# alibasaran/die-e

Measured on AMD Instinct MI355X. Metric: self-play games/sec, higher is better.
Workload: dtype bf16

## Files before the change

### die-e_amd/csrc/mcts_kernels.hip

```cpp
#include <hip/hip_runtime.h>
#include <stdint.h>

#include <algorithm>
#include <type_traits>

#include "bg_device.h"
#include "nn_device.h"
#include "launch.h"
#include "mcts_device.h"
#include "search_types.h"
#include "wave_ops.h"

namespace diee {

__device__ __forceinline__ void backprop(const Tree& T, size_t base, uint32_t idx, float v) {
    while (idx != kNone) {
        T.visits[base + idx] += 1.0f;
        T.value[base + idx] += v;
        idx = T.parent[base + idx];
    }
}

__device__ __forceinline__ void backprop_path(const Tree& T, size_t base, uint32_t my_node, int lane, uint32_t len, float v) {
    if ((uint32_t)lane < len) {
// ... 877 lines not shown
            __syncthreads();
        }
        const uint32_t share = ncand < want ? ncand : want, dem = hit ? 0u : 1u;
        mine_rows = dem + share;
        uint32_t start = 0;
        if (lane == 0 && mine_rows) start = atomicAdd(&L.n_rows[A.q], mine_rows);
        start = (uint32_t)__builtin_amdgcn_readfirstlane((int)start);
        if ((uint32_t)lane < mine_rows && start + (uint32_t)lane < L.rows) {
            const uint32_t node = (dem && lane == 0) ? leaf : D.cand[(uint32_t)lane - dem];
            const uint32_t r = A.q * L.rows + start + (uint32_t)lane;
            store_state(&L.rows_state[r], (dem && lane == 0) ? lst : load_state(&T.state[base + node]));
            L.rows_node[r] = (slot << 24) | node;
        }
        uint32_t extra = 0;
        if (second_round) {
            uint32_t unused_;
            const bool met = tail_meet(L.bar2 + A.q, n, true, lane, S.overflow, unused_);
            const uint32_t more = redistribute ? ncand - share : 0u;
            extra = met ? nchild + more : 0u;
            uint32_t start2 = 0;
            if (lane == 0 && extra) {
                start2 = atomicAdd(&L.n_rows[A.q], extra);
                const uint32_t fit = start2 >= L.rows ? 0u : extra < L.rows - start2 ? extra : L.rows - start2;
                if (fit < extra) atomicSub(&L.n_rows[A.q], extra - fit);
            }
            start2 = (uint32_t)__builtin_amdgcn_readfirstlane((int)start2);
            extra = start2 >= L.rows ? 0u : extra < L.rows - start2 ? extra : L.rows - start2;
            for (uint32_t j = (uint32_t)lane; j < extra; j += 64) {
                const uint32_t r = A.q * L.rows + start2 + j;
                if (j < nchild) {
                    BgState cs = lst;
                    int d0, d1;
                    draw_dice(seed, gid, rnd, it + 1u, j, d0, d1);
                    bg_apply_dev(cs, D.ws.play[j], d0, d1);
                    store_state(&L.rows_state[r], cs);
                    L.rows_node[r] = (slot << 24) | (used + j);
                } else {
                    const uint32_t node = D.cand[share + (j - nchild)];
                    store_state(&L.rows_state[r], load_state(&T.state[base + node]));
                    L.rows_node[r] = (slot << 24) | node;
                }
            }
        }
        cn[SC_NN_ROWS] += mine_rows + extra;
        if (lane == 0 && share + extra) atomicAdd(&L.state[3], share + extra);
    }
    if (lane == 0) store_counters(S, slot, cn);
    TL_STAMP(3);
    if (slot == 0 && lane == 0 && !done) L.n_dem[A.q] = misses;
    if (slot == 0 && lane == 0) {
        const uint32_t was = atomicMax(&L.state[1], done ? 1u : 0u);
        const uint32_t now = was > (done ? 1u : 0u) ? was : (done ? 1u : 0u);
        L.state[0] = it;
        if (!done) L.state[2] += 1u;
        L.host[0] = it; L.host[1] = now; L.host[2] = A.q;
        __threadfence_system();
    }
}

constexpr int kFreeSpinFew = 48, kFreeFewGames = 64;
constexpr uint32_t kFreeRowBits = 12;
struct FreeArgs { Free F; uint32_t q; };
#ifdef DIEE_TAIL_STAMPS
__device__ unsigned long long g_free_stamps[16];
#define FR_STAMP(i) do { const unsigned long long tn_ = __builtin_readcyclecounter(); if (threadIdx.x == 0) atomicAdd(&g_free_stamps[i], tn_ - fr_prev_); fr_prev_ = __builtin_readcyclecounter(); } while (0)
#define FR_COUNT(i, k) do { if (threadIdx.x == 0) atomicAdd(&g_free_stamps[i], (unsigned long long)(k)); } while (0)
extern "C" int diee_dev_free_stamps(unsigned long long* out, int reset) {
    if (out && hipMemcpyFromSymbol(out, HIP_SYMBOL(g_free_stamps), sizeof(unsigned long long) * 16) != hipSuccess) return 1;
    if (reset) { unsigned long long z[16] = {0}; if (hipMemcpyToSymbol(HIP_SYMBOL(g_free_stamps), z, sizeof(z)) != hipSuccess) return 1; }
    return 0;
}
#else
#define FR_STAMP(i) do {} while (0)
#define FR_COUNT(i, k) do {} while (0)
#endif
constexpr uint32_t kFreeLdsNodeBytes = 32;
__host__ __device__ __forceinline__ constexpr uint32_t free_hdr(uint32_t meta, uint32_t first_child) {
    return (meta & 0xE0000000u) | (((meta >> 16) & 0x1ffu) << 20) | (first_child & 0xFFFFFu);
}
__host__ __device__ __forceinline__ constexpr uint32_t hdr_nch(uint32_t h) { return (h >> 20) & 0x1ffu; }
__host__ __device__ __forceinline__ constexpr uint32_t hdr_fc(uint32_t h) { return h & 0xFFFFFu; }
__host__ __device__ constexpr size_t free_lds_bytes(uint32_t ln) {
    return (size_t)ln * kFreeLdsNodeBytes + sizeof(WaveScratch) + sizeof(float) * kMaxPlays + sizeof(uint16_t) * kMaxPlays + sizeof(uint32_t) * 64u;
}
struct TreeF {
    const Tree& T; size_t base; uint32_t ln;
    float *lvis, *lval, *lpri; uint32_t* lhdr;
    __device__ __forceinline__ float vis(uint32_t i) const { return i < ln ? lvis[i] : T.visits[base + i]; }
    __device__ __forceinline__ float val(uint32_t i) const { return i < ln ? lval[i] : T.value[base + i]; }
    __device__ __forceinline__ float pri(uint32_t i) const { return i < ln ? lpri[i] : T.prior[base + i]; }
    __device__ __forceinline__ uint32_t hdr(uint32_t i) const { return i < ln ? lhdr[i] : free_hdr(T.meta[base + i], T.first_child[base + i]); }
    __device__ __forceinline__ void add(uint32_t i, float v) const {
        const float nv = vis(i) + 1.0f, nw = val(i) + v;
        if (i < ln) { lvis[i] = nv; lval[i] = nw; }
        T.visits[base + i] = nv; T.value[base + i] = nw;
    }
    __device__ __forceinline__ void set_header(uint32_t i, uint32_t m, uint32_t f) const {
        if (i < ln) lhdr[i] = free_hdr(m, f);
        T.meta[base + i] = m; T.first_child[base + i] = f;
    }
};
__device__ __forceinline__ uint32_t free_load(const uint32_t* p) { return __hip_atomic_load(p, __ATOMIC_RELAXED, __HIP_MEMORY_SCOPE_AGENT); }

__global__ __launch_bounds__(64) void k_free(Tree T, Slots S, Segs G, uint32_t n, SearchParams P, float c, FreeArgs A) {
    extern __shared__ __attribute__((aligned(16))) char free_smem[];
    const uint32_t slot = blockIdx.x;
    if (slot >= n) return;
    const Free& F = A.F;
    const int lane = threadIdx.x;
    if (F.state[0] != 0u) return;
    uint32_t it = F.prog[slot];
    if (it >= F.iterations) { if (lane == 0) F.wish_n[slot] = it << 8; return; }
    const uint32_t active0 = A.q == 0 ? n : F.state[4];
    const uint32_t active = active0 ? active0 : 1u;
    const bool few = active * 8u <= n || active <= 8u;
    const uint32_t iter_cap = few ? 64u * F.iter_cap : F.iter_cap;
#ifdef DIEE_TAIL_STAMPS
    unsigned long long fr_prev_ = __builtin_readcyclecounter();
    const unsigned long long fr_t0_ = fr_prev_;
#endif
    FR_COUNT(8, 1);
    const uint32_t ln = F.lds_nodes;
    float* lvis = (float*)free_smem; float* lval = lvis + ln; float* lpri = lval + ln;
    float* vvis = lpri + ln; float* vval = vvis + ln;
    float* lcval = vval + ln;
    uint32_t* lhdr = (uint32_t*)(lcval + ln); uint32_t* lcrow = lhdr + ln;
    WaveScratch& ws = *reinterpret_cast<WaveScratch*>(lcrow + ln);
    float* raw = reinterpret_cast<float*>(&ws + 1);
    uint16_t* code = reinterpret_cast<uint16_t*>(raw + kMaxPlays);
    uint32_t* cand = reinterpret_cast<uint32_t*>(code + kMaxPlays);
    float* lgs = (float*)&ws.keyA[0];
    const size_t base = (size_t)slot * T.node_cap;
    uint32_t* crow_g = F.crow + base;
    float* cval_g = F.cval + base;
    const TreeF X{T, base, ln, lvis, lval, lpri, lhdr};
    const bool quirks = P.quirks != 0;
    const uint32_t seg = G.n == 1 ? 0u : S.seg[slot];
    const uint32_t seg_first = G.first_slot[seg], seg_end = G.end_slot[seg];
    const unsigned long long seed = G.seed[seg];
    const uint32_t gid = S.game_id[slot], rnd = S.round[slot];
    const float rv0 = S.root_value0[seg];
    unsigned long long evals = S.counters[(size_t)seg * CNT_COUNT + CNT_NN_EVALS];
    uint32_t used = T.used[slot];
    bool lterm = S.leaf_term[slot] != 0;
    uint32_t leaf = S.leaf[slot], sel = S.sel[slot], leaf_meta = S.leaf_meta[slot];
    float sel_value = S.sel_value[slot];
    uint32_t plen = S.path_len[slot];
    uint32_t pnode = S.path[(size_t)slot * kPathCap + lane];
    uint32_t cn[SC_COUNT];
    load_counters(S, slot, cn);
    const BgState rs = load_state(&T.state[base]);
    const int root_player = st_player(rs);
    uint32_t fsel = 0;
    if (A.q == 0) { if (lane == 0) F.first_sel[slot] = sel == kNone ? kNone : 0u; }
    if (quirks && slot == seg_first) {
        uint32_t m = 0;
        for (uint32_t g = seg_first + (uint32_t)lane; g < seg_end; g += 64) {
            const uint32_t f = A.q == 0 ? (S.sel[g] == kNone ? kNone : 0u) : F.first_sel[g];
            m = f == kNone ? 0x7fffffffu : (f > m ? f : m);
            if (f == kNone) break;
        }
        fsel = (uint32_t)wave_allmax_i32((int)m);
    }
    const uint32_t nl = used < ln ? used : ln;
    for (uint32_t i0 = 0; i0 < nl; i0 += 256) {
        float a[4], b[4], p[4], cv4[4]; uint32_t m[4], f[4], r[4];
#pragma unroll
        for (int u = 0; u < 4; ++u) {
            const uint32_t i = i0 + 64u * u + (uint32_t)lane;
            const size_t gi = base + (i < nl ? i : 0u);
            a[u] = T.visits[gi]; b[u] = T.value[gi]; p[u] = T.prior[gi]; m[u] = T.meta[gi]; f[u] = T.first_child[gi]; r[u] = crow_g[i < nl ? i : 0u]; cv4[u] = cval_g[i < nl ? i : 0u];
        }
#pragma unroll
        for (int u = 0; u < 4; ++u) {
            const uint32_t i = i0 + 64u * u + (uint32_t)lane;
            if (i < nl) { lvis[i] = a[u]; lval[i] = b[u]; lpri[i] = p[u]; lhdr[i] = free_hdr(m[u], f[u]); lcrow[i] = r[u]; lcval[i] = cv4[u]; }
        }
    }
    __syncthreads();
    if (A.q > 0) {
        const uint32_t pq = A.q - 1, off = F.grant_off[slot], cnt = F.grant_cnt[slot];
        const size_t rb = (size_t)(pq % F.ring) * F.rows;
        for (uint32_t r = lane; r < cnt; r += 64) {
            const uint32_t row = off + r;
            const uint32_t node = F.rows_idx[rb + row] - (uint32_t)base;
            const float* h = F.hv + (rb + row) * 72;
            float dot = 0.0f;
            for (int i = 0; i < 72; ++i) dot += h[i] * S.wv[i];
            const float cv = tanhf(dot + S.wv[72]);
            const uint32_t id = ((pq << kFreeRowBits) | row) + 1u;
            cval_g[node] = cv; crow_g[node] = id;
            if (node < ln) { lcrow[node] = id; lcval[node] = cv; }
        }
        cn[SC_NN_ROWS] += cnt;
        __syncthreads();
    }
    auto at_hand = [&](uint32_t cr) { return cr != 0u && ((cr - 1u) >> kFreeRowBits) + F.ring >= A.q; };
    auto crow_of = [&](uint32_t i) { return i < ln ? lcrow[i] : crow_g[i]; };
    auto batch_progress = [&]() {
        int m = 0x7fffffff;
        for (uint32_t g = seg_first + (uint32_t)lane; g < seg_end; g += 64) { const int v = (int)free_load(&F.prog[g]); m = v < m ? v : m; }
        return (uint32_t)(-wave_allmax_i32(-m));
    };
    BgState lst = load_state(&S.eval_states[slot]);
    FR_STAMP(0);
    bool have = false, stalled = false;
    uint32_t minprog = 0;
    auto net_row = [&](uint32_t cr_) {
        NetRowLoaded p;
        const size_t ring = (size_t)(((cr_ - 1u) >> kFreeRowBits) % F.ring) * F.rows + ((cr_ - 1u) & ((1u << kFreeRowBits) - 1u));
        p.vh = value_head_load(F.hv + ring * 72, S.wv, lane);
        softmax_load(F.logits + ring * 1352, lane, p.lg);
        return p;
    };
    uint32_t cr = lterm ? 0u : crow_of(leaf);
    NetRowLoaded pre;
    if (!lterm && at_hand(cr)) pre = net_row(cr);
    uint32_t ran = 0;
    for (;; ++ran) {
        have = lterm || at_hand(cr);
        if (!have) break;
        if (ran >= iter_cap) { stalled = true; break; }
        uint32_t* iflag = S.iter_flags + 2 * ((size_t)seg * G.iter_cap + it);
        const bool need_cnt = quirks && slot == seg_first && it < fsel;
        const bool need_any = lterm && (quirks || slot == seg_first);
        uint2 ifl = make_uint2(1u, 0u);
        if (need_any || need_cnt) {
            bool fin = false;
            const int spins = n <= (uint32_t)kFreeFewGames ? kFreeSpinFew : 1;
            for (int spin = 0; spin < spins; ++spin) {
                if (!need_cnt && (iflag[0] != 0u || free_load(&iflag[0]) != 0u)) { ifl.x = 1u; fin = true; break; }
                if (minprog < it) minprog = batch_progress();
                if (minprog >= it) {
                    ifl.x = free_load(&iflag[0]); ifl.y = free_load(&iflag[1]);
                    fin = true;
                    break;
                }
                __builtin_amdgcn_s_sleep(8);
            }
            if (!fin) { stalled = true; break; }
        }
        FR_STAMP(1);
        const bool active = ifl.x != 0u;
        float v = 0.0f;
        bool do_expand = !lterm, do_backprop = true;
        if (active) {
            if (slot == seg_first) evals += (unsigned long long)(seg_end - seg_first);
            if (lterm) {
                do_expand = false; do_backprop = false;
                if (quirks && sel != kNone) {
                    if (plen) { if ((uint32_t)lane < plen) X.add(pnode, sel_value); }
                    else if (lane == 0) { for (uint32_t i = sel; i != kNone; i = T.parent[base + i]) X.add(i, sel_value); }
                }
            } else {
                v = value_head_eval(pre.vh, lane);
                sel_value = v;
            }
            const uint32_t m0 = lterm ? 0u : leaf_meta;
            if (do_expand && !(m0 & kDrained)) {
                int k = bg_legal_plays_wave(lst, &ws, lane, S.overflow);
                if (k > kMaxPlays) { if (lane == 0) atomicOr(S.overflow, 1u); k = 0; }
                const int r0 = st_roll(lst, 0), r1 = st_roll(lst, 1);
                float smM, smInv;
                softmax_reduce(pre.lg, lane, smM, smInv);
#pragma unroll
                for (int q = 0; q < 22; ++q) lgs[lane + 64 * q] = pre.lg[q];
                __syncthreads();
                for (int j = lane; j < k; j += 64) {
                    const uint32_t cd = bg_encode_dev(r0, r1, ws.play[j]);
                    raw[j] = softmax_prob(lgs[cd], smM, smInv); code[j] = (uint16_t)cd;
                }
                __syncthreads();
                float pr[4];
#pragma unroll
                for (int r = 0; r < 4; ++r) pr[r] = lane + 64 * r < k ? raw[lane + 64 * r] : 0.0f;
                float sum = 0.0f;
#pragma unroll
                for (int r = 0; r < 4; ++r) {
                    const int kr = k - 64 * r < 64 ? k - 64 * r : 64;
                    for (int j = 0; j < kr; ++j) sum += __builtin_bit_cast(float, __builtin_amdgcn_readlane(__builtin_bit_cast(int, pr[r]), j));
                }
                const uint32_t first = used;
                if (first + (uint32_t)k > T.node_cap) {
                    if (lane == 0) atomicOr(S.overflow, 2u);
                } else {
                    const uint32_t e = it + 1u;
                    for (int j = lane; j < k; j += 64) {
                        const uint32_t cl = first + (uint32_t)j;
                        const size_t ci = base + cl;
                        BgState cs = lst;
                        int d0, d1;
                        draw_dice(seed, gid, rnd, e, (uint32_t)j, d0, d1);
                        bg_apply_dev(cs, ws.play[j], d0, d1);
                        store_state(&T.state[ci], cs);
                        const float prj = raw[j] / sum;
                        const uint32_t cm = (uint32_t)code[j] | meta_terminal_bits(cs);
                        T.visits[ci] = 0.0f; T.value[ci] = 0.0f; T.prior[ci] = prj;
                        T.parent[ci] = leaf; T.first_child[ci] = 0; T.meta[ci] = cm;
                        crow_g[cl] = 0u;
                        if (cl < ln) { lvis[cl] = 0.0f; lval[cl] = 0.0f; lpri[cl] = prj; lhdr[cl] = free_hdr(cm, 0u); lcrow[cl] = 0; }
                    }
                    const uint32_t nmeta = kDrained | ((uint32_t)k << 16) | (m0 & kMetaKeep);
                    if (lane == 0) X.set_header(leaf, nmeta, first);
                    used = first + (uint32_t)k;
                    cn[SC_EXPANSIONS] += 1; cn[SC_CHILDREN] += (uint32_t)k;
                    if ((uint32_t)k > cn[SC_MAX_CHILDREN]) cn[SC_MAX_CHILDREN] = (uint32_t)k;
                }
                __syncthreads();
            }
            if (do_backprop) {
                if (plen) { if ((uint32_t)lane < plen) X.add(pnode, v); }
                else if (lane == 0) { for (uint32_t i = leaf; i != kNone; i = T.parent[base + i]) X.add(i, v); }
            }
            if (quirks && slot == seg_first && ifl.y != 0u && lane == 0) {
                float rvis = X.vis(0), rval = X.val(0);
                for (uint32_t i = 0; i < ifl.y; ++i) { rvis += 1.0f; rval += rv0; }
                if (ln > 0) { lvis[0] = rvis; lval[0] = rval; }
                T.visits[base] = rvis; T.value[base] = rval;
            }
            __syncthreads();
        }
        FR_STAMP(2);
        uint32_t published = 0;
        if (it + 1 < F.iterations) {
            uint32_t* nflag = S.iter_flags + 2 * ((size_t)seg * G.iter_cap + it + 1);
            uint32_t node = 0, depth = 0, mine = lane == 0 ? 0u : kNone;
            uint32_t mt = X.hdr(0), fcn = hdr_fc(mt);
            float nvis = X.vis(0);
            for (;;) {
                const uint32_t k = hdr_nch(mt);
                if (k == 0) break;
                const float sq = sqrtf(nvis);
                Best b{0.0f, -1};
                int lastnan = -1;
                for (uint32_t j = lane; j < k; j += 64) {
                    const uint32_t ci = fcn + j;
                    const float vis = X.vis(ci), val = X.val(ci), pr = X.pri(ci);
                    const float q = vis == 0.0f ? 0.0f : val / vis;
                    const float t = sq / (vis + 1.0f);
                    const float u = c * t;
                    const float w = u * pr;
                    const float sc_ = q + w;
                    if (sc_ != sc_) lastnan = (int)j;
                    else if (b.j < 0 || !(b.s > sc_)) { b.s = sc_; b.j = (int)j; }
                }
                lastnan = wave_allmax_i32(lastnan);
                if (lastnan >= 0) {
                    b.s = 0.0f; b.j = -1;
                    for (uint32_t j = lane; j < k; j += 64) {
                        if ((int)j <= lastnan) continue;
                        const uint32_t ci = fcn + j;
                        const float vis = X.vis(ci), val = X.val(ci), pr = X.pri(ci);
                        const float q = vis == 0.0f ? 0.0f : val / vis;
                        const float t = sq / (vis + 1.0f);
                        const float u = c * t;
                        const float w = u * pr;
                        const float sc_ = q + w;
                        if (b.j < 0 || !(b.s > sc_)) { b.s = sc_; b.j = (int)j; }
                    }
                }
                b = wave_best(b);
                const int chosen = b.j >= 0 ? b.j : lastnan;
                node = fcn + (uint32_t)chosen;
                ++depth;
                if ((uint32_t)lane == depth) mine = node;
                mt = X.hdr(node); fcn = hdr_fc(mt); nvis = X.vis(node);
            }
            const uint32_t npl = depth < S.path_cap ? depth + 1u : 0u;
            cn[SC_SELECTIONS] += 1; cn[SC_DEPTH_SUM] += depth;
            if (mt & kMetaTerminal) {
                const float tv = ((mt & kMetaWinnerPlus) ? 1 : -1) == root_player ? 1.0f : -1.0f;
                if (npl) { if ((uint32_t)lane < npl) X.add(mine, tv); }
                else if (lane == 0) { for (uint32_t i = node; i != kNone; i = T.parent[base + i]) X.add(i, tv); }
                cn[SC_TERMINAL] += 1;
                lterm = true;
                if (lane == 0 && quirks && sel == kNone) published = atomicAdd(&nflag[1], 1u);
            } else {
                lterm = false; leaf = node; plen = npl; pnode = mine;
                leaf_meta = T.meta[base + node];
                if (lane == 0) {
                    if (nflag[0] == 0u) published = atomicOr(&nflag[0], 1u);
                    if (sel == kNone) F.first_sel[slot] = it + 1u;
                }
                sel = node;
                lst = load_state(&T.state[base + node]);
            }
            cr = lterm ? 0u : crow_of(leaf);
            if (!lterm && at_hand(cr)) pre = net_row(cr);
        }
        ++it;
        __syncthreads();
        if (lane == 0) {
            asm volatile("" :: "v"(published) : "memory");
            atomicExch(&F.prog[slot], it);
        }
        FR_STAMP(3); FR_COUNT(9, 1);
        if (it >= F.iterations) break;
    }
    if (lane == 0) {
        S.leaf_term[slot] = lterm ? 1 : 0; S.leaf[slot] = leaf; S.sel[slot] = sel; S.leaf_meta[slot] = leaf_meta;
        S.sel_value[slot] = sel_value; S.path_len[slot] = (uint8_t)plen;
        T.used[slot] = used;
        if (slot == seg_first) S.counters[(size_t)seg * CNT_COUNT + CNT_NN_EVALS] = evals;
        store_state(&S.eval_states[slot], lst);
    }
    if ((uint32_t)lane < plen) S.path[(size_t)slot * kPathCap + lane] = pnode;
    const bool done = it >= F.iterations;
    uint32_t nw = 0;
    const bool dem = !done && !stalled && !have;
    if (!done) {
        uint32_t* wl = F.wish + (size_t)slot * kFreeWish;
        if (dem) { if (lane == 0) wl[0] = leaf; nw = 1; }
        uint32_t want0 = F.cand_max < kFreeWish - 1u ? F.cand_max : kFreeWish - 1u;
        uint32_t steps_max = F.rollout_steps;
        if (few && want0) {
            const uint32_t room = (F.rows > active ? F.rows - active : 0u) / active;
            want0 = room + 1u < kFreeWish - 1u ? (room + 1u > want0 ? room + 1u : want0) : kFreeWish - 1u;
            steps_max = 2u * F.rollout_steps + 8u;
        }
        const uint32_t want = few ? want0 : (want0 > ran / 2u + 1u ? want0 - ran / 2u : (want0 ? 1u : 0u));
        uint32_t ncand = 0;
        if (want > 0 && steps_max > 0) {
            const uint32_t nu = used < ln ? used : ln;
            for (uint32_t i = lane; i < nu; i += 64) { vvis[i] = lvis[i]; vval[i] = lval[i]; }
            __syncthreads();
            const uint32_t demanded = dem ? leaf : kNone;
            uint32_t fruitless = 0;
            for (uint32_t step = 0; step < steps_max && ncand < want && fruitless < 8; ++step) {
                uint32_t node = 0, depth = 0, mine = lane == 0 ? 0u : kNone, mt = 0;
                for (;;) {
                    mt = X.hdr(node);
                    const uint32_t k = hdr_nch(mt);
                    if (k == 0) break;
                    const uint32_t fcn = hdr_fc(mt);
                    const float sq = __builtin_amdgcn_sqrtf(node < nu ? vvis[node] : T.visits[base + node]);
                    Best b{0.0f, -1};
                    for (uint32_t j = lane; j < k; j += 64) {
                        const uint32_t ci = fcn + j;
                        const float vis = ci < nu ? vvis[ci] : T.visits[base + ci], val = ci < nu ? vval[ci] : T.value[base + ci];
                        const float q = vis == 0.0f ? 0.0f : val * __builtin_amdgcn_rcpf(vis);
                        const float sc_ = q + (c * (sq * __builtin_amdgcn_rcpf(vis + 1.0f))) * X.pri(ci);
                        if (sc_ == sc_ && (b.j < 0 || !(b.s > sc_))) { b.s = sc_; b.j = (int)j; }
                    }
                    b = wave_best(b);
                    node = fcn + (uint32_t)(b.j >= 0 ? b.j : (int)k - 1);
                    ++depth;
                    if ((uint32_t)lane == depth) mine = node;
                    if (depth >= 63) break;
                }
                const uint32_t cr = crow_of(node);
                float x = 0.0f;
                bool fresh = false;
                if (mt & kMetaTerminal) x = ((mt & kMetaWinnerPlus) ? 1 : -1) == root_player ? 1.0f : -1.0f;
                else if (at_hand(cr)) x = node < ln ? lcval[node] : cval_g[node];
                else if (!(mt & kDrained) && node != demanded) fresh = __ballot((uint32_t)lane < ncand && cand[lane] == node) == 0ull;
                if (fresh) { if (lane == 0) { cand[ncand] = node; wl[nw + ncand] = node; } ++ncand; fruitless = 0; } else ++fruitless;
                if ((uint32_t)lane <= depth && mine < nu) { vvis[mine] += 1.0f; vval[mine] += x; }
                __syncthreads();
                FR_COUNT(11, 1);
            }
        }
        nw += ncand;
    }
    if (lane == 0) {
        F.wish_n[slot] = nw | (it << 8) | (dem ? 0x80000000u : 0u);
        store_counters(S, slot, cn);
    }
    FR_STAMP(4);
#ifdef DIEE_TAIL_STAMPS
    if (threadIdx.x == 0) atomicMax(&g_free_stamps[10], __builtin_readcyclecounter() - fr_t0_);
#endif
}

__global__ __launch_bounds__(1024) void k_free_pack(Free F, uint32_t n, uint32_t node_cap, uint32_t q, const BgState* __restrict__ arena) {
    const uint32_t kBoost = F.lag_boost < kFreeBoostMax ? F.lag_boost : kFreeBoostMax, kLagStep = F.lag_step ? F.lag_step : 1u;
    __shared__ uint32_t hist[kFreeWish + kFreeBoostMax + 2];
    __shared__ uint32_t wsum[16];
    __shared__ uint32_t s_full, s_rem, s_dem, s_undone, s_maxprog;
    const int tid = threadIdx.x, lane = tid & 63, wave = tid >> 6;
    if (F.state[0] != 0u) return;
    if (tid < (int)(kFreeWish + kFreeBoostMax + 2)) hist[tid] = 0;
    if (tid == 0) { s_dem = 0; s_undone = 0; s_maxprog = 0; }
    __syncthreads();
    const uint32_t rot = (q * 131u) % n;
    const uint32_t g = (uint32_t)tid < n ? ((uint32_t)tid + rot) % n : 0u;
    const uint32_t w = (uint32_t)tid < n ? F.wish_n[g] : ((F.iterations) << 8);
    const uint32_t cnt = (w & 0xffu) < kFreeWish ? (w & 0xffu) : kFreeWish, dem = (w >> 31) < cnt ? (w >> 31) : cnt, spec = cnt - dem, prog = (w >> 8) & 0x7fffffu;
    const bool undone = prog < F.iterations;
    if ((uint32_t)tid < n && undone) { atomicMax(&s_maxprog, prog); atomicAdd(&s_undone, 1u); if (dem) atomicAdd(&s_dem, 1u); }
    __syncthreads();
    const uint32_t lag = undone ? s_maxprog - prog : 0u;
    const uint32_t shift = kBoost - (lag / kLagStep < kBoost ? lag / kLagStep : kBoost);
    if ((uint32_t)tid < n) for (uint32_t r = 1; r <= spec; ++r) atomicAdd(&hist[r + shift], 1u);
    __syncthreads();
    if (tid == 0) {
        const uint32_t room = F.rows > s_dem ? F.rows - s_dem : 0u;
        uint32_t full = 0, used_rows = 0;
        for (uint32_t k = 1; k <= kFreeWish + kBoost; ++k) {
            if (used_rows + hist[k] > room) break;
            used_rows += hist[k]; full = k;
        }
        s_full = full; s_rem = room - used_rows;
    }
    __syncthreads();
    const uint32_t full = s_full, rem = s_rem;
    const uint32_t whole = full > shift ? (full - shift < spec ? full - shift : spec) : 0u;
    const int more = ((uint32_t)tid < n && spec > whole && whole + 1u + shift == full + 1u) ? 1 : 0;
    int inc = wave_inclusive_scan_i32(more);
    if (lane == 63) wsum[wave] = (uint32_t)inc;
    __syncthreads();
    uint32_t before = 0;
    for (int v = 0; v < wave; ++v) before += wsum[v];
    const uint32_t my_rank = before + (uint32_t)(inc - more);
    __syncthreads();
    const uint32_t grant = (uint32_t)tid < n ? dem + whole + ((more && my_rank < rem) ? 1u : 0u) : 0u;
    inc = wave_inclusive_scan_i32((int)grant);
    if (lane == 63) wsum[wave] = (uint32_t)inc;
    __syncthreads();
    before = 0;
    uint32_t total = 0;
    for (int v = 0; v < 16; ++v) { if (v < wave) before += wsum[v]; total += wsum[v]; }
    const uint32_t off = before + (uint32_t)inc - grant;
    if ((uint32_t)tid < n) {
        const uint32_t fit = off >= F.rows ? 0u : (grant < F.rows - off ? grant : F.rows - off);
        F.grant_off[g] = off; F.grant_cnt[g] = fit;
        uint32_t* out = F.rows_idx + (size_t)(q % F.ring) * F.rows + off;
        const uint32_t* wl = F.wish + (size_t)g * kFreeWish;
        for (uint32_t j = 0; j < fit; ++j) out[j] = g * node_cap + wl[j];
        if (F.rows_state) {
            BgState* so = F.rows_state + (size_t)(q % F.ring) * F.rows + off;
            for (uint32_t j = 0; j < fit; ++j) store_state(&so[j], load_state(&arena[(size_t)g * node_cap + wl[j]]));
        }
    }
    if (tid == 0) {
        if (total > F.rows) total = F.rows;
        F.n_rows[q] = total; F.n_dem[q] = s_dem < total ? s_dem : total;
        const uint32_t all_done = s_undone ? 0u : 1u;
        F.state[0] = all_done; F.state[4] = s_undone;
        if (total) { F.state[1] += 1u; F.state[2] += total - s_dem; }
        F.host[0] = all_done; F.host[1] = q;
        __threadfence_system();
    }
}

__global__ __launch_bounds__(256) void k_reduce_counters(Slots S, Segs G, unsigned long long* step_log, uint32_t step) {
    __shared__ unsigned long long part[SC_COUNT][4];
    const uint32_t seg = blockIdx.x;
    const uint32_t s0 = G.first_slot[seg], s1 = G.end_slot[seg];
    if (s1 <= s0) return;
    const int tid = threadIdx.x, lane = tid & 63, wave = tid >> 6;
    unsigned long long acc[SC_COUNT];
#pragma unroll
    for (int c = 0; c < SC_COUNT; ++c) acc[c] = 0;
    for (uint32_t s = s0 + tid; s < s1; s += 256)
#pragma unroll
        for (int c = 0; c < SC_COUNT; ++c) {
            const unsigned long long v = S.slot_cnt[s * SC_COUNT + c];
            if (c == SC_MAX_CHILDREN) acc[c] = v > acc[c] ? v : acc[c]; else acc[c] += v;
        }
#pragma unroll
    for (int c = 0; c < SC_COUNT; ++c) {
#pragma unroll
        for (int d = 32; d >= 1; d >>= 1) {
            const unsigned long long o = __shfl_xor(acc[c], d);
            if (c == SC_MAX_CHILDREN) acc[c] = o > acc[c] ? o : acc[c]; else acc[c] += o;
        }
        if (lane == 0) part[c][wave] = acc[c];
    }
    __syncthreads();
    if (tid == 0) {
        const int map[SC_COUNT] = {CNT_SELECTIONS, CNT_DEPTH_SUM, CNT_TERMINAL, CNT_EXPANSIONS, CNT_CHILDREN, CNT_MAX_CHILDREN, CNT_ILLEGAL, CNT_NN_ROWS};
        unsigned long long* cnt = S.counters + (size_t)seg * CNT_COUNT;
        for (int c = 0; c < SC_COUNT; ++c) {
            unsigned long long t = 0;
            for (int w = 0; w < 4; ++w) t = c == SC_MAX_CHILDREN ? (part[c][w] > t ? part[c][w] : t) : t + part[c][w];
            if (c == SC_MAX_CHILDREN) { if (t > cnt[map[c]]) cnt[map[c]] = t; }
            else cnt[map[c]] += t;
            if (step_log && c == SC_EXPANSIONS) atomicAdd(&step_log[2 * (size_t)step], t);
            if (step_log && c == SC_NN_ROWS) atomicAdd(&step_log[2 * (size_t)step + 1], t);
        }
    }
}

__global__ __launch_bounds__(1024) void k_row_map(const uint8_t* __restrict__ skip, uint32_t n, uint32_t* __restrict__ row_slot,
                                                  uint32_t* __restrict__ slot_row, uint32_t* __restrict__ n_rows,
                                                  uint32_t* __restrict__ rows_log, uint32_t log_idx) {
    __shared__ uint32_t wsum[16];
    __shared__ uint32_t carry;
    const int tid = threadIdx.x, lane = tid & 63, wave = tid >> 6;
    if (tid == 0) carry = 0;
    __syncthreads();
    for (uint32_t c0 = 0; c0 < n; c0 += 1024) {
        const uint32_t i = c0 + tid;
        const bool keep = i < n && skip[i] == 0;
        const unsigned long long bal = __ballot(keep);
        if (lane == 0) wsum[wave] = (uint32_t)__popcll(bal);
        __syncthreads();
        uint32_t off = carry;
        for (int w = 0; w < wave; ++w) off += wsum[w];
        const uint32_t pos = off + (uint32_t)__popcll(bal & ((1ull << lane) - 1ull));
        if (keep) { row_slot[pos] = i; slot_row[i] = pos; }
        __syncthreads();
        if (tid == 0) { uint32_t t = 0; for (int w = 0; w < 16; ++w) t += wsum[w]; carry += t; }
        __syncthreads();
    }
    if (tid == 0) { *n_rows = carry; if (rows_log) rows_log[log_idx] = carry; }
}

__global__ __launch_bounds__(64) void k_root_probs(Tree T, uint32_t n, float* __restrict__ probs,
                                                   uint32_t* __restrict__ nch, float* __restrict__ root_visits) {
    __shared__ float sum_s;
    const uint32_t slot = blockIdx.x;
    if (slot >= n) return;
    const int lane = threadIdx.x;
    const size_t base = (size_t)slot * T.node_cap;
    const uint32_t k = meta_nch(T.meta[base]), fc = T.first_child[base];
    float* row = probs + (size_t)slot * 1352;
    const float fill = k == 0 ? __uint_as_float(0x7fc00000u) : 0.0f;
    for (int a = lane; a < 1352; a += 64) row[a] = fill;
    if (lane == 0) {
        float s = 0.0f;
        for (uint32_t j = 0; j < k; ++j) s += T.visits[base + fc + j];
        sum_s = s;
        nch[slot] = k;
// ... 118 lines not shown
        Gm.rounds[g] = round + 1;
        atomicAdd(&cnt[CNT_PLIES], 1ull);
        const int w = bg_winner_dev(s);
        if (w != 0) {
            if (!(flushed && !P.quirks)) { Gm.ev_b_count[g] = nf + 1; Gm.ev_b_step[g] = step; }
            Gm.winner[g] = (int8_t)w;
            removed = true;
        }
        if (removed) { Gm.alive[g] = 0; atomicAdd(&cnt[CNT_GAMES], 1ull); }
    }
}

__global__ __launch_bounds__(1024) void k_compact_live(Games Gm, uint32_t n_live, uint32_t n_segs, uint32_t* n_live_out) {
    __shared__ uint32_t wsum[16];
    __shared__ uint32_t carry;
    __shared__ uint32_t per_seg[kMaxSegments];
    const int tid = threadIdx.x, lane = tid & 63, wave = tid >> 6;
    if (tid == 0) carry = 0;
    if (tid < (int)kMaxSegments) per_seg[tid] = 0;
    __syncthreads();
    for (uint32_t c0 = 0; c0 < n_live; c0 += 1024) {
        const uint32_t i = c0 + tid;
        uint32_t g = 0;
        bool keep = false;
        if (i < n_live) { g = Gm.live[i]; keep = Gm.alive[g] != 0; }
        if (keep) atomicAdd(&per_seg[Gm.seg[g]], 1u);
        const unsigned long long bal = __ballot(keep);
        if (lane == 0) wsum[wave] = (uint32_t)__popcll(bal);
        __syncthreads();
        uint32_t off = carry;
        for (int w = 0; w < wave; ++w) off += wsum[w];
        const uint32_t pos = off + (uint32_t)__popcll(bal & ((1ull << lane) - 1ull));
        __syncthreads();
        if (keep) Gm.live[pos] = g;
        __syncthreads();
        if (tid == 0) { uint32_t t = 0; for (int w = 0; w < 16; ++w) t += wsum[w]; carry += t; }
        __syncthreads();
    }
    if (tid == 0) n_live_out[0] = carry;
    if (tid < (int)n_segs) n_live_out[1 + tid] = per_seg[tid];
}

__global__ __launch_bounds__(1024) void k_deliver_scan(Games Gm, Segs G, uint32_t n_live, uint32_t step, DeliverEvent* __restrict__ ev,
                                                       uint32_t* __restrict__ summary) {
    __shared__ uint32_t wrow[16], wev[16];
    __shared__ uint32_t carry_rows, carry_ev;
    __shared__ uint32_t seg_base[kMaxSegments], seg_rows[kMaxSegments], seg_ev0[kMaxSegments], seg_nev[kMaxSegments];
    const int tid = threadIdx.x, lane = tid & 63, wave = tid >> 6;
    if (tid == 0) { carry_rows = 0; carry_ev = 0; }
    if (tid < (int)kMaxSegments) { seg_base[tid] = 0; seg_rows[tid] = 0; seg_ev0[tid] = kNone; seg_nev[tid] = 0; }
    __syncthreads();
    for (uint32_t c0 = 0; c0 < n_live; c0 += 1024) {
        const uint32_t i = c0 + tid;
        uint32_t g = 0, seg = 0, ca = 0, cb = 0;
        if (i < n_live) {
            g = Gm.live[i]; seg = Gm.seg[g];
            const uint32_t a = Gm.ev_a_count[g], b = Gm.ev_b_count[g];
            if (a != kNone && Gm.ev_a_step[g] == step) ca = a;
            if (b != kNone && Gm.ev_b_step[g] == step) cb = b;
        }
        const uint32_t nr = ca + cb, ne = (ca ? 1u : 0u) + (cb ? 1u : 0u);
        uint32_t pr = nr, pe = ne;
#pragma unroll
        for (int d = 1; d < 64; d <<= 1) {
            const uint32_t xr = __shfl_up(pr, d, 64), xe = __shfl_up(pe, d, 64);
            if (lane >= d) { pr += xr; pe += xe; }
        }
        if (lane == 63) { wrow[wave] = pr; wev[wave] = pe; }
        __syncthreads();
        uint32_t off_r = carry_rows, off_e = carry_ev;
        for (int w = 0; w < wave; ++w) { off_r += wrow[w]; off_e += wev[w]; }
        const uint32_t row0 = off_r + pr - nr;
        uint32_t e = off_e + pe - ne;
        if (i < n_live && i == G.first_slot[seg]) seg_base[seg] = row0;
        if (ca) { ev[e] = DeliverEvent{g, ca, row0, seg}; ++e; }
        if (cb) ev[e] = DeliverEvent{g, 0x80000000u | cb, row0 + ca, seg};
        __syncthreads();
        if (tid == 0) { uint32_t tr = 0, te = 0; for (int w = 0; w < 16; ++w) { tr += wrow[w]; te += wev[w]; } carry_rows += tr; carry_ev += te; }
        __syncthreads();
    }
    const uint32_t n_ev = carry_ev;
    for (uint32_t e = tid; e < n_ev; e += 1024) {
        DeliverEvent d = ev[e];
        d.row0 -= seg_base[d.seg];
        ev[e] = d;
        atomicAdd(&seg_rows[d.seg], d.kind_count & 0x7FFFFFFFu);
        atomicMin(&seg_ev0[d.seg], e);
        atomicAdd(&seg_nev[d.seg], 1u);
    }
    __syncthreads();
    if (tid < (int)G.n) {
        summary[DeliverSummary::rows(G.n, tid)] = seg_rows[tid];
        summary[DeliverSummary::ev0(G.n, tid)] = seg_nev[tid] ? seg_ev0[tid] : 0u;
        summary[DeliverSummary::nev(G.n, tid)] = seg_nev[tid];
    }
}

__global__ __launch_bounds__(256) void k_deliver_copy(Games Gm, Segs G, const DeliverEvent* __restrict__ ev, uint32_t n_ev, uint32_t r0,
                                                      uint32_t r1, DeliverOut out) {
    for (uint32_t r = r0 + blockIdx.x; r < r1; r += gridDim.x) {
        uint32_t lo = 0, hi = n_ev;
        while (hi - lo > 1) { const uint32_t mid = (lo + hi) >> 1; if (ev[mid].row0 <= r) lo = mid; else hi = mid; }
        const DeliverEvent d = ev[lo];
        const uint32_t fr = r - d.row0;
        const size_t s = (size_t)d.g * Gm.frag_cap + fr, o = (size_t)(r - r0);
        for (int a = threadIdx.x; a < 1352 / 4; a += 256)
            reinterpret_cast<float4*>(out.ps + o * 1352)[a] = reinterpret_cast<const float4*>(Gm.frag_ps + s * 1352)[a];
        if (threadIdx.x < 144 / 4)
            reinterpret_cast<float4*>(out.planes + o * 144)[threadIdx.x] = reinterpret_cast<const float4*>(Gm.frag_planes + s * 144)[threadIdx.x];
        if (threadIdx.x == 0) {
            const int pl = Gm.frag_player[s], w = Gm.winner[d.g];
            out.outcome[o] = (d.kind_count >> 31) == 0 ? (int8_t)0 : (int8_t)(w == pl ? 1 : (w == -pl ? -1 : 0));
            out.game[o] = G.first_id[d.seg] + (d.g - G.game0[d.seg]);
        }
    }
}

void launch_init_roots(hipStream_t st, const Tree& T, const Slots& S, uint32_t n) {
    hipLaunchKernelGGL(k_init_roots, dim3((n + 255) / 256), dim3(256), 0, st, T, S, n);
}
void launch_expand(hipStream_t st, const Tree& T, const Slots& S, const Segs& G, uint32_t n, uint32_t it, const SearchParams& P,
                   uint32_t next_it, float c, bool pre_grown, ExpandVariant v) {
    if (pre_grown && v.two_c) hipLaunchKernelGGL((k_expand<true, 2>), dim3(n), dim3(128), 0, st, T, S, G, n, it, P, next_it, c);
    else if (pre_grown) hipLaunchKernelGGL((k_expand<true, 0>), dim3(n), dim3(64), 0, st, T, S, G, n, it, P, next_it, c);
    else if (v.two) hipLaunchKernelGGL((k_expand<true, 1>), dim3(n), dim3(128), 0, st, T, S, G, n, it, P, next_it, c);
    else hipLaunchKernelGGL((k_expand<false, 0>), dim3(n), dim3(64), 0, st, T, S, G, n, it, P, next_it, c);
}
void launch_tail(hipStream_t st, const Tree& T, const Slots& S, const Segs& G, uint32_t n, const SearchParams& P, float c, const Tail& L, uint32_t q) {
    static bool attr_set[16] = {};
    int dev = 0;
    (void)hipGetDevice(&dev);
    if (!attr_set[dev & 15]) {
        (void)hipFuncSetAttribute((const void*)k_tail, hipFuncAttributeMaxDynamicSharedMemorySize, (int)sizeof(TailLds));
        attr_set[dev & 15] = true;
    }
    hipLaunchKernelGGL(k_tail, dim3(n <= 32 ? 8 * n : n), dim3(64), sizeof(TailLds), st, T, S, G, n, P, c, TailArgs{L, q});
}
uint32_t free_lds_nodes_for(uint32_t n, uint32_t cus) {
    const uint32_t per_cu = (n + cus - 1) / (cus ? cus : 1u);
    const size_t budget = (size_t)160 * 1024 / (per_cu ? per_cu : 1u);
    const size_t fixed = free_lds_bytes(0);
    if (budget <= fixed + 64 * kFreeLdsNodeBytes) return 64;
    uint32_t ln = (uint32_t)((budget - fixed) / kFreeLdsNodeBytes) / 64 * 64;
    return ln > kTailLdsNodes ? kTailLdsNodes : ln;
}
void launch_free(hipStream_t st, const Tree& T, const Slots& S, const Segs& G, uint32_t n, const SearchParams& P, float c, const Free& F, uint32_t q) {
    static bool attr_set[16] = {};
    int dev = 0;
    (void)hipGetDevice(&dev);
    if (!attr_set[dev & 15]) {
        (void)hipFuncSetAttribute((const void*)k_free, hipFuncAttributeMaxDynamicSharedMemorySize, (int)free_lds_bytes(kTailLdsNodes));
        attr_set[dev & 15] = true;
    }
    hipLaunchKernelGGL(k_free, dim3(n), dim3(64), free_lds_bytes(F.lds_nodes), st, T, S, G, n, P, c, FreeArgs{F, q});
    hipLaunchKernelGGL(k_free_pack, dim3(1), dim3(1024), 0, st, F, n, T.node_cap, q, T.state);
}
void launch_reduce_counters(hipStream_t st, const Slots& S, const Segs& G, unsigned long long* step_log, uint32_t step) {
    hipLaunchKernelGGL(k_reduce_counters, dim3(G.n), dim3(256), 0, st, S, G, step_log, step);
}
void launch_row_map(hipStream_t st, const uint8_t* skip, uint32_t n, uint32_t* row_slot, uint32_t* slot_row, uint32_t* n_rows,
                    uint32_t* rows_log, uint32_t log_idx) {
    hipLaunchKernelGGL(k_row_map, dim3(1), dim3(1024), 0, st, skip, n, row_slot, slot_row, n_rows, rows_log, log_idx);
}
void launch_root_probs(hipStream_t st, const Tree& T, uint32_t n, float* probs, uint32_t* nch, float* root_visits) {
    hipLaunchKernelGGL(k_root_probs, dim3(n), dim3(64), 0, st, T, n, probs, nch, root_visits);
}
void launch_init_games(hipStream_t st, const Games& Gm, const Segs& G, uint32_t n) {
    hipLaunchKernelGGL(k_init_games, dim3((n + 255) / 256), dim3(256), 0, st, Gm, G, n);
}
void launch_gather_roots(hipStream_t st, const Games& Gm, const Slots& S, const Segs& G, uint32_t n_live) {
    hipLaunchKernelGGL(k_gather_roots, dim3((n_live + 255) / 256), dim3(256), 0, st, Gm, S, G, n_live);
}
void launch_play_move(hipStream_t st, const Tree& T, const Games& Gm, const Segs& G, uint32_t n_live, uint32_t step, const PlayParams& P) {
    hipLaunchKernelGGL(k_play_move, dim3(n_live), dim3(64), 0, st, T, Gm, G, n_live, step, P);
}
void launch_compact_live(hipStream_t st, const Games& Gm, uint32_t n_live, uint32_t n_segs, uint32_t* n_live_out) {
    hipLaunchKernelGGL(k_compact_live, dim3(1), dim3(1024), 0, st, Gm, n_live, n_segs, n_live_out);
}
void launch_deliver_scan(hipStream_t st, const Games& Gm, const Segs& G, uint32_t n_live, uint32_t step, DeliverEvent* ev, uint32_t* summary) {
    hipLaunchKernelGGL(k_deliver_scan, dim3(1), dim3(1024), 0, st, Gm, G, n_live, step, ev, summary);
}
void launch_deliver_copy(hipStream_t st, const Games& Gm, const Segs& G, const DeliverEvent* ev, uint32_t n_ev, uint32_t r0, uint32_t r1,
                         const DeliverOut& out) {
    if (r1 <= r0 || !n_ev) return;
    hipLaunchKernelGGL(k_deliver_copy, dim3(std::min<uint32_t>(r1 - r0, 8192u)), dim3(256), 0, st, Gm, G, ev, n_ev, r0, r1, out);
}

}
```

Measured before the change: 120.7.

## Add LDS-resident single-pass selection fast paths in free-search kernel

```diff
diff --git a/die-e_amd/csrc/mcts_kernels.hip b/die-e_amd/csrc/mcts_kernels.hip
--- a/die-e_amd/csrc/mcts_kernels.hip
+++ b/die-e_amd/csrc/mcts_kernels.hip
@@ -1053,11 +1053,10 @@
     const BgState rs = load_state(&T.state[base]);
     const int root_player = st_player(rs);
     uint32_t fsel = 0;
-    if (A.q == 0) { if (lane == 0) F.first_sel[slot] = sel == kNone ? kNone : 0u; }
     if (quirks && slot == seg_first) {
         uint32_t m = 0;
         for (uint32_t g = seg_first + (uint32_t)lane; g < seg_end; g += 64) {
-            const uint32_t f = A.q == 0 ? (S.sel[g] == kNone ? kNone : 0u) : F.first_sel[g];
+            const uint32_t f = F.first_sel[g];
             m = f == kNone ? 0x7fffffffu : (f > m ? f : m);
             if (f == kNone) break;
         }
@@ -1232,6 +1231,29 @@
                 const uint32_t k = hdr_nch(mt);
                 if (k == 0) break;
                 const float sq = sqrtf(nvis);
+                if (k <= 64u && fcn + k <= ln) {
+                    const bool valid = (uint32_t)lane < k;
+                    const uint32_t ci = fcn + (valid ? (uint32_t)lane : 0u);
+                    const float vis = lvis[ci], val = lval[ci], pr = lpri[ci];
+                    const uint32_t ch = lhdr[ci];
+                    const float q = vis == 0.0f ? 0.0f : val / vis;
+                    const float t = sq / (vis + 1.0f);
+                    const float u = c * t;
+                    const float w = u * pr;
+                    const float sc_ = q + w;
+                    const unsigned long long nans = __ballot(valid && sc_ != sc_);
+                    const int lastnan = nans ? 63 - __clzll((long long)nans) : -1;
+                    const bool comp = valid && sc_ == sc_ && lane > lastnan;
+                    const float mx = wave_allmax_f32(comp ? sc_ : -INFINITY);
+                    const unsigned long long win = __ballot(comp && sc_ == mx);
+                    const int chosen = win ? 63 - __clzll((long long)win) : lastnan;
+                    node = fcn + (uint32_t)chosen;
+                    ++depth;
+                    if ((uint32_t)lane == depth) mine = node;
+                    mt = (uint32_t)__builtin_amdgcn_readlane((int)ch, chosen); fcn = hdr_fc(mt);
+                    nvis = __builtin_bit_cast(float, __builtin_amdgcn_readlane(__builtin_bit_cast(int, vis), chosen));
+                    continue;
+                }
                 Best b{0.0f, -1};
                 int lastnan = -1;
                 for (uint32_t j = lane; j < k; j += 64) {
@@ -1323,10 +1345,92 @@
         uint32_t ncand = 0;
         if (want > 0 && steps_max > 0) {
             const uint32_t nu = used < ln ? used : ln;
-            for (uint32_t i = lane; i < nu; i += 64) { vvis[i] = lvis[i]; vval[i] = lval[i]; }
+            for (uint32_t i0 = 0; i0 < nu; i0 += 256) {
+                float a[4], b[4];
+#pragma unroll
+                for (int u = 0; u < 4; ++u) { const uint32_t i = i0 + 64u * u + (uint32_t)lane; a[u] = lvis[i < nu ? i : 0u]; b[u] = lval[i < nu ? i : 0u]; }
+#pragma unroll
+                for (int u = 0; u < 4; ++u) { const uint32_t i = i0 + 64u * u + (uint32_t)lane; if (i < nu) { vvis[i] = a[u]; vval[i] = b[u]; } }
+            }
             __syncthreads();
             const uint32_t demanded = dem ? leaf : kNone;
             uint32_t fruitless = 0;
+            const uint32_t h0 = X.hdr(0), k0 = hdr_nch(h0), fc0 = hdr_fc(h0);
+            const bool resident = used <= ln && k0 >= 1u && k0 <= 64u;
+            if (resident) {
+                auto rl_u = [](uint32_t v_, int l_) { return (uint32_t)__builtin_amdgcn_readlane((int)v_, l_); };
+                auto rl_f = [](float v_, int l_) { return __builtin_bit_cast(float, __builtin_amdgcn_readlane(__builtin_bit_cast(int, v_), l_)); };
+                const bool rc = (uint32_t)lane < k0;
+                const uint32_t rci = fc0 + (rc ? (uint32_t)lane : 0u);
+                float r_vis = vvis[0], c_vis = vvis[rci], c_val = vval[rci];
+                const float c_pri = lpri[rci], c_cval = lcval[rci];
+                const uint32_t c_hdr = lhdr[rci], c_crow = lcrow[rci];
+                uint32_t my_cand = kNone;
+                for (uint32_t step = 0; step < steps_max && ncand < want && fruitless < 8; ++step) {
+                    auto last_max = [&](bool comp, float sc_, uint32_t k_) {
+                        const float mx = wave_allmax_f32(comp ? sc_ : -INFINITY);
+                        const unsigned long long win = __ballot(comp && sc_ == mx);
+                        return win ? 63 - __clzll((long long)win) : (int)k_ - 1;
+                    };
+                    int j0;
+                    {
+                        const float sq = __builtin_amdgcn_sqrtf(r_vis);
+                        const float q = c_vis == 0.0f ? 0.0f : c_val * __builtin_amdgcn_rcpf(c_vis);
+                        const float sc_ = q + (c * (sq * __builtin_amdgcn_rcpf(c_vis + 1.0f))) * c_pri;
+                        j0 = last_max(rc && sc_ == sc_, sc_, k0);
+                    }
+                    uint32_t node = fc0 + (uint32_t)j0, depth = 1, mine = kNone, mt = h0;
+                    uint32_t hn = rl_u(c_hdr, j0), ncr = rl_u(c_crow, j0);
+                    float pvis = rl_f(c_vis, j0), pval = 0.0f, ncv = rl_f(c_cval, j0), mvis = 0.0f, mval = 0.0f;
+                    for (;;) {
+                        mt = hn;
+                        const uint32_t k = hdr_nch(mt);
+                        if (k == 0) break;
+                        const uint32_t fcn = hdr_fc(mt);
+                        const float sq = __builtin_amdgcn_sqrtf(pvis);
+                        if (k <= 64u) {
+                            const bool valid = (uint32_t)lane < k;
+                            const uint32_t ci = fcn + (valid ? (uint32_t)lane : 0u);
+                            const float vis = vvis[ci], val = vval[ci], pr = lpri[ci], cv = lcval[ci];
+                            const uint32_t h = lhdr[ci], cr = lcrow[ci];
+                            const float q = vis == 0.0f ? 0.0f : val * __builtin_amdgcn_rcpf(vis);
+                            const float sc_ = q + (c * (sq * __builtin_amdgcn_rcpf(vis + 1.0f))) * pr;
+                            const int lw = last_max(valid && sc_ == sc_, sc_, k);
+                            node = fcn + (uint32_t)lw;
+                            hn = rl_u(h, lw); ncr = rl_u(cr, lw); pvis = rl_f(vis, lw); pval = rl_f(val, lw); ncv = rl_f(cv, lw);
+                            ++depth;
+                            if ((uint32_t)lane == depth) { mine = node; mvis = pvis; mval = pval; }
+                            if (depth >= 63) break;
+                            continue;
+                        }
+                        Best b{0.0f, -1};
+                        for (uint32_t j = lane; j < k; j += 64) {
+                            const uint32_t ci = fcn + j;
+                            const float vis = vvis[ci], val = vval[ci];
+                            const float q = vis == 0.0f ? 0.0f : val * __builtin_amdgcn_rcpf(vis);
+                            const float sc_ = q + (c * (sq * __builtin_amdgcn_rcpf(vis + 1.0f))) * lpri[ci];
+                            if (sc_ == sc_ && (b.j < 0 || !(b.s > sc_))) { b.s = sc_; b.j = (int)j; }
+                        }
+                        b = wave_best(b);
+                        node = fcn + (uint32_t)(b.j >= 0 ? b.j : (int)k - 1);
+                        hn = lhdr[node]; ncr = lcrow[node]; pvis = vvis[node]; pval = vval[node]; ncv = lcval[node];
+                        ++depth;
+                        if ((uint32_t)lane == depth) { mine = node; mvis = pvis; mval = pval; }
+                        if (depth >= 63) break;
+                    }
+                    float x = 0.0f;
+                    bool fresh = false;
+                    if (mt & kMetaTerminal) x = ((mt & kMetaWinnerPlus) ? 1 : -1) == root_player ? 1.0f : -1.0f;
+                    else if (at_hand(ncr)) x = ncv;
+                    else if (!(mt & kDrained) && node != demanded) fresh = __ballot((uint32_t)lane < ncand && my_cand == node) == 0ull;
+                    if (fresh) { if ((uint32_t)lane == ncand) my_cand = node; if (lane == 0) wl[nw + ncand] = node; ++ncand; fruitless = 0; } else ++fruitless;
+                    r_vis += 1.0f;
+                    if (lane == j0) { c_vis += 1.0f; c_val += x; }
+                    if (lane >= 2 && (uint32_t)lane <= depth) { vvis[mine] = mvis + 1.0f; vval[mine] = mval + x; }
+                    __builtin_amdgcn_wave_barrier();
+                    FR_COUNT(11, 1);
+                }
+            } else
             for (uint32_t step = 0; step < steps_max && ncand < want && fruitless < 8; ++step) {
                 uint32_t node = 0, depth = 0, mine = lane == 0 ? 0u : kNone, mt = 0;
                 for (;;) {
@@ -1371,6 +1475,11 @@
 #ifdef DIEE_TAIL_STAMPS
     if (threadIdx.x == 0) atomicMax(&g_free_stamps[10], __builtin_readcyclecounter() - fr_t0_);
 #endif
+}
+
+__global__ __launch_bounds__(256) void k_free_first_sel(const uint32_t* __restrict__ sel, uint32_t* __restrict__ first_sel, uint32_t n) {
+    const uint32_t g = blockIdx.x * 256u + threadIdx.x;
+    if (g < n) first_sel[g] = sel[g] == kNone ? kNone : 0u;
 }
 
 __global__ __launch_bounds__(1024) void k_free_pack(Free F, uint32_t n, uint32_t node_cap, uint32_t q, const BgState* __restrict__ arena) {
@@ -1795,6 +1904,7 @@
         (void)hipFuncSetAttribute((const void*)k_free, hipFuncAttributeMaxDynamicSharedMemorySize, (int)free_lds_bytes(kTailLdsNodes));
         attr_set[dev & 15] = true;
     }
+    if (q == 0) hipLaunchKernelGGL(k_free_first_sel, dim3((n + 255u) / 256u), dim3(256), 0, st, S.sel, F.first_sel, n);
     hipLaunchKernelGGL(k_free, dim3(n), dim3(64), free_lds_bytes(F.lds_nodes), st, T, S, G, n, P, c, FreeArgs{F, q});
     hipLaunchKernelGGL(k_free_pack, dim3(1), dim3(1024), 0, st, F, n, T.node_cap, q, T.state);
 }
```

Result: faster. 123.6 (median of 6 runs) (+2.4%).
